# anonymousauthors001/SGS-GNN

Measured on AMD Instinct MI355X. Metric: sampled edges/sec + training steps/sec, Reddit hybrid 20% sparsity, higher is better.
Workload: dtype f32

## Files before the change

include/sgs_hip.h:

```cpp
#ifndef SGS_HIP_H_
#define SGS_HIP_H_

#include <stddef.h>
#include <stdint.h>

#ifdef __cplusplus
extern "C" {
#endif

#define SGS_ABI_VERSION 1

#define SGS_OK 0
#define SGS_EINVAL (-1)
#define SGS_EWORKSPACE (-2)
#define SGS_EHIP (-3)

typedef void* sgs_stream_t;

int sgs_abi_version(void);
const char* sgs_last_error(void);

int sgs_rng_set_epoch_buffer(const uint64_t* epoch_dev);
int sgs_exp_noise(uint64_t seed, uint64_t stream_id, int64_t E, float* noise, sgs_stream_t stream);
int sgs_dropout_keep(uint64_t seed, uint32_t site, int64_t rows, int64_t cols, float p, uint8_t* keep,
// ... 66 lines not shown

int sgs_gcn_norm_fwd(const float* w, int64_t n_edges, int64_t N, const int32_t* in_ptr, const int32_t* in_src,
                     const int32_t* in_eid, const int32_t* out_ptr, const int32_t* out_dst, const int32_t* out_eid,
                     const int32_t* loop_eid, float* dis, float* loopw, float* what_in, float* what_out,
                     float* what_loop, sgs_stream_t stream);

int sgs_gcn_degree_partial(const float* w, int64_t n_edges, int64_t N, const int32_t* in_ptr, const int32_t* in_src,
                           const int32_t* in_eid, float* degpart, sgs_stream_t stream);
int sgs_gcn_norm_from_degree(const float* w, const float* degsum, int64_t n_edges, int64_t N, const int32_t* in_ptr,
                             const int32_t* in_src, const int32_t* in_eid, const int32_t* out_ptr,
                             const int32_t* out_dst, const int32_t* out_eid, float* dis, float* loopw, float* what_in,
                             float* what_out, float* what_loop, sgs_stream_t stream);
int sgs_bias_act(const float* X, const float* bias, int64_t N, int64_t D, int act, float p_drop, uint64_t seed,
                 uint32_t site, float* Y, sgs_stream_t stream);
int sgs_bias_act_rows(const float* X, const float* bias, int64_t n_rows, int64_t D, int64_t row_offset, int act, float p_drop,
                      uint64_t seed, uint32_t site, float* Y, sgs_stream_t stream);

int sgs_mean_weights(int64_t n_edges, int64_t N, const int32_t* in_ptr, const int32_t* out_ptr, const int32_t* out_dst,
                     float* what_in, float* what_out, sgs_stream_t stream);
int sgs_degree_prior_logits(const int64_t* edge_index, int64_t E, int64_t N, const int32_t* in_ptr,
                            const int32_t* out_ptr, float* logits, sgs_stream_t stream);

size_t sgs_gcn_norm_bwd_workspace_bytes(int64_t N);
int sgs_gcn_norm_bwd(const float* w, const float* gw_hat, const float* gloop, int64_t n_edges, int64_t N,
                     const float* dis, const float* loopw, const int32_t* in_ptr, const int32_t* in_src,
                     const int32_t* in_eid, const int32_t* out_ptr, const int32_t* out_dst, const int32_t* out_eid,
                     const int32_t* loop_eid, const int64_t* edge_index, float* dw, void* ws, size_t ws_bytes,
                     sgs_stream_t stream);
int sgs_gcn_norm_bwd_sum(const float* w, const float* gw_hat, const float* gloop, const float* gw_hat2, const float* gloop2, const float* dw_add,
                         int64_t n_edges, int64_t N, const float* dis, const float* loopw, const int32_t* in_ptr, const int32_t* in_src,
                         const int32_t* in_eid, const int32_t* out_ptr, const int32_t* out_dst, const int32_t* out_eid,
                         const int32_t* loop_eid, const int64_t* edge_index, float* dw, void* ws, size_t ws_bytes, sgs_stream_t stream);

int sgs_gcn_norm_bwd_node(const float* w, const float* gw_hat, const float* gloop, int64_t n_edges, int64_t N,
                          const float* dis, const float* loopw, const int32_t* in_ptr, const int32_t* in_src,
                          const int32_t* in_eid, const int32_t* out_ptr, const int32_t* out_dst, const int32_t* out_eid,
                          float* Hn, sgs_stream_t stream);
int sgs_gcn_norm_bwd_edge(const float* gw_hat, const float* gloop, int64_t n_edges, int64_t N, const float* dis,
                          const int32_t* loop_eid, const int64_t* edge_index, const float* Hn, float* dw,
                          sgs_stream_t stream);

#define SGS_ACT_NONE 0
#define SGS_ACT_RELU 1
#define SGS_ACT_RELU_DROPOUT 2
int sgs_spmm_csr(const float* X, int64_t N, int64_t D, int64_t nnz, const int32_t* ptr, const int32_t* col, const float* val,
                 const float* diag, const float* bias, int act, float p_drop, uint64_t seed, uint32_t site, float* Y,
                 sgs_stream_t stream);

int sgs_sddmm_csr(const float* A, const float* B, int64_t N, int64_t D, int64_t nnz, const int32_t* ptr, const int32_t* col,
                  const int32_t* eid, float* g, float* gdiag, sgs_stream_t stream);

int sgs_spmm_csr_variant(int64_t N, int64_t D, int64_t nnz, int aligned16);
int sgs_sddmm_csr_variant(int64_t N, int64_t D, int64_t nnz, int aligned16);

int sgs_spmm_long_rows_set(int on);
int sgs_spmm_long_rows_threshold(void);
int sgs_spmm_long_rows_active(int64_t N, int64_t D);

int sgs_act_bwd(const float* dY, const float* Y, int64_t n, int act, float p_drop, float* dZ, sgs_stream_t stream);
size_t sgs_colsum_workspace_bytes(int64_t N, int64_t D);
int sgs_colsum(const float* A, int64_t N, int64_t D, float* out, void* ws, size_t ws_bytes, sgs_stream_t stream);
int sgs_act_bwd_colsum(const float* dY, const float* Y, int64_t N, int64_t D, int act, float p_drop, float* dZ, float* colsum, void* ws,
                       size_t ws_bytes, sgs_stream_t stream);

int sgs_colsum_variant(int64_t N, int64_t D, int fused_act);

int sgs_gcn_pair_ok(int64_t N, int64_t nnz, int64_t D);
int sgs_spmm_csr_next(const float* X, int64_t N, int64_t D, int64_t nnz, const int32_t* ptr, const int32_t* col, const float* val,
                      const float* diag, const float* bias, int act, float p_drop, uint64_t seed, uint32_t site, const float* Wn, int64_t Dn,
                      float* Y, float* Z, sgs_stream_t stream);
int sgs_spmm_csr_bwd_prev(const float* dZ, int64_t N, int64_t D, int64_t nnz, const int32_t* ptr, const int32_t* col, const float* val,
                          const float* diag, const float* W, int64_t Dp, const float* Yp, int act, float p_drop, float* dX, float* dZp,
                          float* colsum, sgs_stream_t stream);

int sgs_gcn_dual_ok(int64_t N, int64_t nnz_a, int64_t nnz_b, int64_t D, int64_t Dn);
int sgs_spmm_csr_next_dual(const float* X, int64_t N, int64_t D, const float* bias, int act, float p_drop, uint32_t site, const float* Wn,
                           int64_t Dn, int64_t nnz_a, const int32_t* ptr_a, const int32_t* col_a, const float* val_a, const float* diag_a,
                           uint64_t seed_a, float* Y_a, float* Z_a, int64_t nnz_b, const int32_t* ptr_b, const int32_t* col_b,
                           const float* val_b, const float* diag_b, uint64_t seed_b, float* Y_b, float* Z_b, sgs_stream_t stream);
int sgs_spmm_csr_dual(const float* X_a, const float* X_b, int64_t N, int64_t D, const float* bias, int act, float p_drop, uint32_t site,
                      int64_t nnz_a, const int32_t* ptr_a, const int32_t* col_a, const float* val_a, const float* diag_a, uint64_t seed_a,
                      float* Y_a, int64_t nnz_b, const int32_t* ptr_b, const int32_t* col_b, const float* val_b, const float* diag_b,
                      uint64_t seed_b, float* Y_b, sgs_stream_t stream);

size_t sgs_edge_score_workspace_bytes(int64_t N, int64_t H, int64_t E);
int sgs_edge_score_hidden_supported(int64_t H);
int sgs_edge_score_get_variant(void);
int sgs_edge_score_get_bwd_variant(void);
void sgs_edge_score_set_bwd_variant(int variant);
int sgs_edge_score_bwd_tile(void);
void sgs_edge_score_set_variant(int variant);
int sgs_edge_score_fwd(const float* codes, const float* U, int64_t N, int64_t H, const int64_t* edge_index, int64_t E,
                       int64_t edge_id_offset, const float* W1, const float* b1, const float* w2, const float* b2,
                       float p_drop, uint64_t seed, uint32_t site, float* p_out, void* ws, size_t ws_bytes,
                       sgs_stream_t stream);
size_t sgs_edge_mates_workspace_bytes(int64_t n_edges);
int sgs_edge_mates(const int64_t* edge_index, int64_t n_edges, int64_t N, const int32_t* out_ptr, const int32_t* out_dst,
                   const int32_t* out_eid, int32_t* mate, void* ws, size_t ws_bytes, sgs_stream_t stream);
int sgs_edge_score_paired_supported(int64_t H);
int sgs_edge_score_fwd_paired(const float* codes, const float* U, int64_t N, int64_t H, const int64_t* edge_index, int64_t E,
                              int64_t edge_id_offset, const int32_t* canon, int64_t M, const int32_t* mate, const float* W1, const float* b1,
                              const float* w2, const float* b2, float p_drop, uint64_t seed, uint32_t site, float* p_out, void* ws,
                              size_t ws_bytes, sgs_stream_t stream);
int sgs_edge_score_bwd_core(const float* codes, const float* U, int64_t N, int64_t H, const int64_t* edge_index,
                            int64_t E, int64_t edge_id_offset, const int64_t* active_eid, int64_t n_active, const float* grad_p,
                            const float* W1, const float* b1, const float* w2, const float* b2, float p_drop,
// ... 356 lines not shown
```

sgs-gnn_amd/csrc/gcn.hip:

```cpp
#include "sgs_common.h"

namespace sgs {
size_t graph_sort_workspace_bytes(int64_t n, int64_t N);
size_t graph_src_sorted_workspace_bytes(int64_t n, int64_t N);
int graph_build_src_sorted(const int64_t* ei, int64_t n, int64_t N, int32_t* in_ptr, int32_t* in_src, int32_t* in_eid, int32_t* out_ptr,
                           int32_t* out_dst, int32_t* out_eid, int32_t* loop_eid, int32_t* unsorted_flag, void* ws, size_t ws_bytes,
                           hipStream_t stream);
int graph_build_by_sort(const int64_t* ei, int64_t n, int64_t N, int32_t* in_ptr, int32_t* in_src, int32_t* in_eid, int32_t* out_ptr,
                        int32_t* out_dst, int32_t* out_eid, int32_t* loop_eid, void* ws, size_t ws_bytes, hipStream_t stream);
}

namespace sgs {
namespace {

constexpr int kT = 256;
constexpr int kMaxLdsRow = 8192;

__global__ void __launch_bounds__(kT) count_degrees(const int64_t* __restrict__ ei, int64_t n_edges, int* __restrict__ cnt_in,
                                                   int* __restrict__ cnt_out, int* __restrict__ loop_eid) {
    const int64_t e = static_cast<int64_t>(blockIdx.x) * kT + threadIdx.x;
    if (e >= n_edges) return;
    const int s = static_cast<int>(ei[e]), d = static_cast<int>(ei[n_edges + e]);
    atomicAdd(&cnt_in[d], 1);
    atomicAdd(&cnt_out[s], 1);
// ... 801 lines not shown
        float a[VEC];
#pragma unroll
        for (int v = 0; v < VEC; ++v) a[v] = 0.f;
        if (in) *reinterpret_cast<V*>(a) = *reinterpret_cast<const V*>(Ai + c0);
        const int64_t cl = in ? c0 : 0;
        for (int k = b + wave; k < e; k += 4 * NW) {
            int jc[4], ev[4];
#pragma unroll
            for (int u = 0; u < 4; ++u) {
                const int kk = k + NW * u;
                const int kc = kk < e ? kk : e - 1;
                jc[u] = col[kc];
                ev[u] = eid[kc];
            }
            float x[4][VEC];
#pragma unroll
            for (int u = 0; u < 4; ++u) *reinterpret_cast<V*>(x[u]) = *reinterpret_cast<const V*>(B + static_cast<int64_t>(jc[u]) * D + cl);
            float d[4];
#pragma unroll
            for (int u = 0; u < 4; ++u) {
                float acc = 0.f;
#pragma unroll
                for (int v = 0; v < VEC; ++v) acc = fmaf(a[v], in ? x[u][v] : 0.f, acc);
                d[u] = acc;
            }
#pragma unroll
            for (int u = 0; u < 4; ++u) d[u] = wave_sum_hi_dpp(d[u]);
            if (lane == 63) {
#pragma unroll
                for (int u = 0; u < 4; ++u)
                    if (k + NW * u < e) g[ev[u]] = d[u];
            }
        }
        if (wave == 0 && gdiag) {
            const float d0 = wave_sum_all(dot(i));
            if (lane == 0) gdiag[i] = d0;
        }
        return;
    }
    int k = b + wave;
    for (; k + NW < e; k += 2 * NW) {
        float d0 = dot(col[k]), d1 = dot(col[k + NW]);
#pragma unroll
        for (int o = 32; o > 0; o >>= 1) { d0 += __shfl_xor(d0, o, 64); d1 += __shfl_xor(d1, o, 64); }
        if (lane == 0) { g[eid[k]] = d0; g[eid[k + NW]] = d1; }
    }
    for (; k < e; k += NW) {
        const float d0 = wave_sum_all(dot(col[k]));
        if (lane == 0) g[eid[k]] = d0;
    }
    if (wave == 0 && gdiag) {
        const float d0 = wave_sum_all(dot(i));
        if (lane == 0) gdiag[i] = d0;
    }
}

__global__ void __launch_bounds__(kT) act_bwd(const float* __restrict__ dY, const float* __restrict__ Y, int64_t n, int act,
                                             float drop_scale, float* __restrict__ dZ) {
    const int64_t i = static_cast<int64_t>(blockIdx.x) * kT + threadIdx.x;
    if (i >= n) return;
    float g = dY[i];
    if (act != SGS_ACT_NONE) g = (Y[i] > 0.f) ? (act == SGS_ACT_RELU_DROPOUT ? g * drop_scale : g) : 0.f;
    dZ[i] = g;
}

constexpr int kColRows = 256;
inline int colsum_rows(int64_t N) { return N >= 16384 ? kColRows : (N >= 4096 ? 128 : 32); }
__global__ void __launch_bounds__(kT) colsum_partial(const float* __restrict__ A, int64_t N, int64_t D, int rows, float* __restrict__ part) {
    __shared__ float red[4][64];
    const int c = blockIdx.x * 64 + (threadIdx.x & 63);
    const int rgrp = threadIdx.x >> 6;
    const int64_t r0 = static_cast<int64_t>(blockIdx.y) * rows;
    const int64_t r1 = (r0 + rows < N) ? r0 + rows : N;
    float acc = 0.f;
    if (c < D)
        for (int64_t r = r0 + rgrp; r < r1; r += 4) acc += A[r * D + c];
    red[rgrp][threadIdx.x & 63] = acc;
    __syncthreads();
    if (rgrp == 0 && c < D)
        part[static_cast<int64_t>(blockIdx.y) * D + c] = (red[0][threadIdx.x] + red[1][threadIdx.x]) + (red[2][threadIdx.x] + red[3][threadIdx.x]);
}
template <int RG>
__global__ void __launch_bounds__(RG * 64) colsum_final(const float* __restrict__ part, int64_t nchunk, int64_t D, float* __restrict__ out) {
    __shared__ float red[RG][64];
    const int c = blockIdx.x * 64 + (threadIdx.x & 63);
    const int rgrp = threadIdx.x >> 6;
    float acc = 0.f;
    if (c < D)
        for (int64_t r = rgrp; r < nchunk; r += RG) acc += part[r * D + c];
    red[rgrp][threadIdx.x & 63] = acc;
    __syncthreads();
    if (rgrp == 0 && c < D) {
        float s = 0.f;
#pragma unroll
        for (int g = 0; g < RG; g += 4) s += (red[g][threadIdx.x] + red[g + 1][threadIdx.x]) + (red[g + 2][threadIdx.x] + red[g + 3][threadIdx.x]);
        out[c] = s;
    }
}

constexpr int kColSmallRows = 2048;
template <bool ACT>
__device__ __forceinline__ void colsum_small_body(const float* __restrict__ A, const float* __restrict__ Y, int64_t N, int64_t D, int act,
                                                  float drop_scale, float* __restrict__ dZ, float* __restrict__ out, int64_t blk) {
    __shared__ float red[64][17];
    const int cl = threadIdx.x & 15, rl = threadIdx.x >> 4;
    const int64_t c = blk * 16 + cl;
// ... 713 lines not shown
    const float scale = 1.0f / (1.0f - p_drop);
    const uint32_t th = dropout_thresh(p_drop);
    if (act == SGS_ACT_RELU_DROPOUT && p_drop == 0.f) act = SGS_ACT_RELU;
    const dim3 g_(static_cast<unsigned>(N));
    const bool lr = spmm_long_rows_on(N, D);
    switch (var) {
        case 1416:
            LAUNCH_LR(spmm_csr_rowblock, 4, 16, g_, dim3(1024), 0, stream, X, N, D, ptr, col, val, diag, bias, act, scale, th, seed,
                               site, epoch_ptr(), Y);
            break;
        case 1404:
            LAUNCH_LR(spmm_csr_rowblock, 4, 4, g_, dim3(kT), 0, stream, X, N, D, ptr, col, val, diag, bias, act, scale, th, seed,
                               site, epoch_ptr(), Y);
            break;
        case 1116:
            LAUNCH_LR(spmm_csr_rowblock, 1, 16, g_, dim3(1024), 0, stream, X, N, D, ptr, col, val, diag, bias, act, scale, th, seed,
                               site, epoch_ptr(), Y);
            break;
        case 1104:
            LAUNCH_LR(spmm_csr_rowblock, 1, 4, g_, dim3(kT), 0, stream, X, N, D, ptr, col, val, diag, bias, act, scale, th, seed,
                               site, epoch_ptr(), Y);
            break;
        default: {
            const int vec = var / 100, lpr = var % 100;
            DISPATCH_VEC_LPR(spmm_csr, vec, lpr, N, X, N, D, ptr, col, val, diag, bias, act, scale, th, seed, site, epoch_ptr(), Y);
        }
    }
    SGS_LAUNCH_OK();
    return SGS_OK;
}

int sgs_sddmm_csr(const float* A, const float* B, int64_t N, int64_t D, int64_t nnz, const int32_t* ptr, const int32_t* col,
                  const int32_t* eid, float* g, float* gdiag, sgs_stream_t stream_) {
    hipStream_t stream = static_cast<hipStream_t>(stream_);
    SGS_REQUIRE(N >= 0 && D >= 0, SGS_EINVAL, "sgs_sddmm_csr: bad sizes");
    if (N == 0) return SGS_OK;
    SGS_REQUIRE(A && B && ptr, SGS_EINVAL, "sgs_sddmm_csr: null pointer");
    const int var = sgs_sddmm_csr_variant(N, D, nnz, aligned16(A) && aligned16(B));
    const dim3 g_(static_cast<unsigned>(N));
    switch (var) {
        case 1416: hipLaunchKernelGGL((sddmm_csr_rowblock<4, 16>), g_, dim3(1024), 0, stream, A, B, N, D, ptr, col, eid, g, gdiag); break;
        case 1404: hipLaunchKernelGGL((sddmm_csr_rowblock<4, 4>), g_, dim3(kT), 0, stream, A, B, N, D, ptr, col, eid, g, gdiag); break;
        case 1116: hipLaunchKernelGGL((sddmm_csr_rowblock<1, 16>), g_, dim3(1024), 0, stream, A, B, N, D, ptr, col, eid, g, gdiag); break;
        case 1104: hipLaunchKernelGGL((sddmm_csr_rowblock<1, 4>), g_, dim3(kT), 0, stream, A, B, N, D, ptr, col, eid, g, gdiag); break;
        default: {
            const int vec = var / 100, lpr = var % 100;
            DISPATCH_VEC_LPR(sddmm_csr, vec, lpr, N, A, B, N, D, ptr, col, eid, g, gdiag);
        }
    }
    SGS_LAUNCH_OK();
    return SGS_OK;
}

int sgs_act_bwd(const float* dY, const float* Y, int64_t n, int act, float p_drop, float* dZ, sgs_stream_t stream_) {
    hipStream_t stream = static_cast<hipStream_t>(stream_);
    SGS_REQUIRE(n >= 0 && p_drop >= 0.f && p_drop < 1.f, SGS_EINVAL, "sgs_act_bwd: bad arguments");
    if (n == 0) return SGS_OK;
    SGS_REQUIRE(dY && dZ && (act == SGS_ACT_NONE || Y), SGS_EINVAL, "sgs_act_bwd: null pointer");
    if (act == SGS_ACT_RELU_DROPOUT && p_drop == 0.f) act = SGS_ACT_RELU;
    hipLaunchKernelGGL(act_bwd, dim3(cdiv(n, kT)), dim3(kT), 0, stream, dY, Y, n, act, 1.0f / (1.0f - p_drop), dZ);
    SGS_LAUNCH_OK();
    return SGS_OK;
}

size_t sgs_colsum_workspace_bytes(int64_t N, int64_t D) {
    if (N < 0) N = 0;
    if (D < 0) D = 0;
    return carve_bytes(static_cast<size_t>(cdiv(N, colsum_rows(N)) + 1) * D, 4) + 256;
}

int sgs_colsum_variant(int64_t N, int64_t D, int fused_act) {
    const int f = fused_act ? 100000 : 0;
    if (N > 0 && N <= kColSmallRows) return (D % 4 == 0 ? 2000000 : 1000000) + f;
    if (D == 1 && N > 0 && N <= kVecSumMax) return 3000000 + f;
    const int rows = colsum_rows(N);
    return 4000000 + f + rows * 100 + (cdiv(N, rows) > 64 ? 16 : 4);
}

int sgs_colsum(const float* A, int64_t N, int64_t D, float* out, void* ws, size_t ws_bytes, sgs_stream_t stream_) {
    hipStream_t stream = static_cast<hipStream_t>(stream_);
    SGS_REQUIRE(N >= 0 && D >= 0, SGS_EINVAL, "sgs_colsum: bad sizes");
    if (D == 0) return SGS_OK;
    SGS_REQUIRE(out && (N == 0 || A), SGS_EINVAL, "sgs_colsum: null pointer");
    SGS_REQUIRE(ws && ws_bytes >= sgs_colsum_workspace_bytes(N, D), SGS_EWORKSPACE, "sgs_colsum: workspace too small");
    const int var = sgs_colsum_variant(N, D, 0);
    switch (var / 1000000) {
        case 1:
            hipLaunchKernelGGL(colsum_small<false>, dim3(cdiv(D, 16)), dim3(1024), 0, stream, A, static_cast<const float*>(nullptr), N, D, SGS_ACT_NONE, 1.f,
                               static_cast<float*>(nullptr), out);
            break;
        case 2:
            hipLaunchKernelGGL(colsum_small_v4<false>, dim3(cdiv(D, 16)), dim3(1024), 0, stream, A, static_cast<const float*>(nullptr), N, D, SGS_ACT_NONE,
                               1.f, static_cast<float*>(nullptr), out);
            break;
        case 3:
            hipLaunchKernelGGL(vecsum_small, dim3(1), dim3(1024), 0, stream, A, N, out);
            break;
        default: {
            Carver cv(ws);
            const int rows = var / 100 % 1000;
            const int64_t nchunk = cdiv(N, rows);
            float* part = cv.take<float>(static_cast<size_t>(nchunk + 1) * D);
            if (nchunk > 0)
                hipLaunchKernelGGL(colsum_partial, dim3(cdiv(D, 64), nchunk), dim3(kT), 0, stream, A, N, D, rows, part);
            if (var % 100 == 16) hipLaunchKernelGGL(colsum_final<16>, dim3(cdiv(D, 64)), dim3(1024), 0, stream, part, nchunk, D, out);
            else                 hipLaunchKernelGGL(colsum_final<4>, dim3(cdiv(D, 64)), dim3(kT), 0, stream, part, nchunk, D, out);
// ... 277 lines not shown
```

sgs-gnn_amd/csrc/optim.hip:

```cpp
#include "sgs_common.h"

namespace sgs {
namespace {

constexpr int kAT = 256;
constexpr int kAChunk = 2048;
constexpr int kAMax = 24;

struct AdamDesc {
    float* p;
    const float* g;
    float* m;
    float* v;
    int64_t n;
    float* step;
    const float* gate;
};
struct AdamArgs {
    AdamDesc d[kAMax];
    int chunk_end[kAMax];
    int n_tensors;
    float lr, beta1, beta2, eps, weight_decay;
    int maximize;
    unsigned int* ticket;
};

__global__ void __launch_bounds__(kAT) adam_group(AdamArgs a) {
    __shared__ unsigned int s_last;
    int ti = 0;
    while (static_cast<int>(blockIdx.x) >= a.chunk_end[ti]) ++ti;
    const int chunk = static_cast<int>(blockIdx.x) - (ti ? a.chunk_end[ti - 1] : 0);
    const AdamDesc d = a.d[ti];
    const bool open = d.gate == nullptr || d.gate[0] != 0.f;
    const float t = d.step[0] + 1.0f;
    const double bc1 = 1.0 - exp(static_cast<double>(t) * log(static_cast<double>(a.beta1)));
    const double bc2 = 1.0 - exp(static_cast<double>(t) * log(static_cast<double>(a.beta2)));
    const float step_size = static_cast<float>(static_cast<double>(a.lr) / bc1);
    const float inv_sqrt_bc2 = static_cast<float>(1.0 / sqrt(bc2));
    const float beta1 = a.beta1, beta2 = a.beta2, eps = a.eps, wd = a.weight_decay;
    const int64_t base = static_cast<int64_t>(chunk) * kAChunk;
#pragma unroll
    for (int it = 0; it < kAChunk / kAT; ++it) {
        const int64_t i = base + static_cast<int64_t>(it) * kAT + threadIdx.x;
        if (open && i < d.n) {
            float g = d.g[i];
            if (a.maximize) g = -g;
            const float p = d.p[i];
            if (wd != 0.f) g = fmaf(wd, p, g);
            float m = d.m[i], v = d.v[i];
            m = m + (g - m) * (1.0f - beta1);
            v = beta2 * v + (1.0f - beta2) * g * g;
            const float denom = sqrtf(v) * inv_sqrt_bc2 + eps;
            d.m[i] = m;
            d.v[i] = v;
            d.p[i] = p - step_size * (m / denom);
        }
    }
    __syncthreads();
    if (threadIdx.x == 0) s_last = (atomicAdd(a.ticket, 1u) == gridDim.x - 1) ? 1u : 0u;
    __syncthreads();
    if (s_last) {
        if (static_cast<int>(threadIdx.x) < a.n_tensors) {
            const AdamDesc& dd = a.d[threadIdx.x];
            if (dd.gate == nullptr || dd.gate[0] != 0.f) dd.step[0] += 1.0f;
        }
        if (threadIdx.x == 0) __hip_atomic_store(a.ticket, 0u, __ATOMIC_RELAXED, __HIP_MEMORY_SCOPE_AGENT);
    }
}

constexpr int kAMax2 = 16;
struct AdamState {
    float* m;
    float* v;
    float* step;
    const float* gate;
    float lr, beta1, beta2, eps, wd;
    int maximize;
};
struct AdamDesc2 {
    float* p;
    const float* g;
    int64_t n;
    AdamState s[2];
    int n_states;
};
struct AdamArgs2 {
    AdamDesc2 d[kAMax2];
    int chunk_end[kAMax2];
    int n_tensors;
    unsigned int* ticket;
    float* loss_sum;
    const float* loss;
    unsigned long long* epoch;
};

__global__ void __launch_bounds__(kAT) adam_multi(AdamArgs2 a) {
    __shared__ unsigned int s_last;
    int ti = 0;
    while (static_cast<int>(blockIdx.x) >= a.chunk_end[ti]) ++ti;
    const int chunk = static_cast<int>(blockIdx.x) - (ti ? a.chunk_end[ti - 1] : 0);
    const AdamDesc2& d = a.d[ti];
    bool open[2];
    float step_size[2], inv_sqrt_bc2[2];
#pragma unroll
    for (int q = 0; q < 2; ++q) {
        open[q] = q < d.n_states && (d.s[q].gate == nullptr || d.s[q].gate[0] != 0.f);
        step_size[q] = 0.f;
        inv_sqrt_bc2[q] = 0.f;
        if (q < d.n_states) {
            const float t = d.s[q].step[0] + 1.0f;
            const double bc1 = 1.0 - exp(static_cast<double>(t) * log(static_cast<double>(d.s[q].beta1)));
            const double bc2 = 1.0 - exp(static_cast<double>(t) * log(static_cast<double>(d.s[q].beta2)));
            step_size[q] = static_cast<float>(static_cast<double>(d.s[q].lr) / bc1);
            inv_sqrt_bc2[q] = static_cast<float>(1.0 / sqrt(bc2));
        }
    }
    const int64_t base = static_cast<int64_t>(chunk) * kAChunk;
#pragma unroll
    for (int it = 0; it < kAChunk / kAT; ++it) {
        const int64_t i = base + static_cast<int64_t>(it) * kAT + threadIdx.x;
        if (i < d.n && (open[0] || open[1])) {
            const float g0 = d.g[i];
            float p = d.p[i];
#pragma unroll
            for (int q = 0; q < 2; ++q) {
                if (open[q]) {
                    const AdamState& st = d.s[q];
                    float g = st.maximize ? -g0 : g0;
                    if (st.wd != 0.f) g = fmaf(st.wd, p, g);
                    float m = st.m[i], v = st.v[i];
                    m = m + (g - m) * (1.0f - st.beta1);
                    v = st.beta2 * v + (1.0f - st.beta2) * g * g;
                    const float denom = sqrtf(v) * inv_sqrt_bc2[q] + st.eps;
                    st.m[i] = m;
                    st.v[i] = v;
                    p = p - step_size[q] * (m / denom);
                }
            }
            d.p[i] = p;
        }
    }
    __syncthreads();
    if (threadIdx.x == 0) s_last = (atomicAdd(a.ticket, 1u) == gridDim.x - 1) ? 1u : 0u;
    __syncthreads();
    if (s_last) {
        if (static_cast<int>(threadIdx.x) < 2 * a.n_tensors) {
            const AdamDesc2& dd = a.d[threadIdx.x >> 1];
            const int q = threadIdx.x & 1;
            if (q < dd.n_states && (dd.s[q].gate == nullptr || dd.s[q].gate[0] != 0.f)) {
                dd.s[q].step[0] += 1.0f;
            }
        }
        if (threadIdx.x == 64) {
            if (a.loss_sum && a.loss) a.loss_sum[0] += a.loss[0];
            if (a.epoch) a.epoch[0] += 1ull;
        }
        if (threadIdx.x == 0) __hip_atomic_store(a.ticket, 0u, __ATOMIC_RELAXED, __HIP_MEMORY_SCOPE_AGENT);
    }
}

}
}

using namespace sgs;

extern "C" {

int sgs_adam_max_tensors(void) { return kAMax; }

int sgs_adam_step(const int64_t* desc_host, int64_t n_tensors, float lr, float beta1, float beta2, float eps, float weight_decay,
                  int maximize, uint32_t* ticket, sgs_stream_t stream_) {
    hipStream_t stream = static_cast<hipStream_t>(stream_);
    SGS_REQUIRE(n_tensors >= 0 && n_tensors <= kAMax, SGS_EINVAL, "sgs_adam_step: at most %d tensors per call", kAMax);
    if (n_tensors == 0) return SGS_OK;
    SGS_REQUIRE(desc_host && ticket, SGS_EINVAL, "sgs_adam_step: null pointer");
    SGS_REQUIRE(beta1 >= 0.f && beta1 < 1.f && beta2 >= 0.f && beta2 < 1.f && eps >= 0.f, SGS_EINVAL, "sgs_adam_step: bad hyper-parameters");
    AdamArgs a{};
    int64_t total = 0;
    for (int i = 0; i < kAMax; ++i) {
        if (i < n_tensors) {
            const int64_t* w = desc_host + 7 * i;
            a.d[i].p = reinterpret_cast<float*>(w[0]);
            a.d[i].g = reinterpret_cast<const float*>(w[1]);
            a.d[i].m = reinterpret_cast<float*>(w[2]);
            a.d[i].v = reinterpret_cast<float*>(w[3]);
            a.d[i].n = w[4];
            a.d[i].step = reinterpret_cast<float*>(w[5]);
            a.d[i].gate = reinterpret_cast<const float*>(w[6]);
            SGS_REQUIRE(a.d[i].p && a.d[i].g && a.d[i].m && a.d[i].v && a.d[i].step && a.d[i].n >= 0, SGS_EINVAL,
                        "sgs_adam_step: bad descriptor %d", i);
            total += cdiv(a.d[i].n, kAChunk);
        }
        a.chunk_end[i] = static_cast<int>(total);
    }
// ... 59 lines not shown
```

sgs-gnn_amd/ops.py:

```python
from __future__ import annotations

import ctypes
import os
from typing import NamedTuple, Optional

import numpy as np
import torch

from . import _lib

SAMPLE_LEARNED, SAMPLE_PRIOR = 0, 1
ACT_NONE, ACT_RELU, ACT_RELU_DROPOUT = 0, 1, 2

_workspaces = {}
_retired_workspaces = []
_pin_workspaces = False


def _need_gpu(*tensors):
    for t in tensors:
        if t is not None and not t.is_cuda:
            raise RuntimeError("sgs_gnn_amd: the SGS hot path runs only on a HIP device (got a CPU tensor); "
                               "there is no CPU fallback")

# ... 1936 lines not shown
    return _leaf_dw(dY, x.contiguous(), x.shape[0], M, Nn, leaf=leaf)


class _GCNLayer(torch.autograd.Function):

    @staticmethod
    def forward(ctx, x, W, handle, bias, nm, act, p, seed, site, xl):
        gr = nm.graph
        if xl is None:
            xl = _x_wt(x, W)
        N, D = xl.shape
        Y = _spmm(xl, gr.in_ptr, gr.in_src, nm.what_in, nm.what_loop, bias, act, p, seed, site, N, D, gr.n_edges)
        ctx.nm, ctx.act, ctx.p = nm, act, p
        ctx.has_bias, ctx.has_handle = bias is not None, handle is not None
        ctx.save_for_backward(x, W, xl, Y if act != ACT_NONE else None)
        ctx.mark_non_differentiable(xl)
        ctx.set_materialize_grads(False)
        return Y, xl

    @staticmethod
    def backward(ctx, dY, _dxl_unused):
        L = _lib.lib()
        nm, gr = ctx.nm, ctx.nm.graph
        x, W, xl, Y = ctx.saved_tensors
        N, D = xl.shape
        dY = dY.contiguous()
        dx = dW = g = None
        want_db = ctx.has_bias and ctx.needs_input_grad[3]
        dZ, dbias = _grad_through_act(dY, Y, ctx.act, ctx.p, want_db, colsum_now=False)
        need_x, need_W = ctx.needs_input_grad[0], ctx.needs_input_grad[1]
        if need_x or need_W:
            dxl = _spmm(dZ, gr.out_ptr, gr.out_dst, nm.what_out, nm.what_loop, None, ACT_NONE, 0.0, 0, 0, N, D, gr.n_edges)
            if need_W:
                dW = _dyt_x(dxl, x, W.shape, leaf=(ctx, 1))
            if need_x:
                dx = dxl @ W
        if ctx.has_handle and ctx.needs_input_grad[2]:
            g = torch.empty(gr.n_edges + gr.N, dtype=torch.float32, device=dY.device)
            gw, gl = g[:gr.n_edges], g[gr.n_edges:]
            _lib.check(L.sgs_sddmm_csr(_ptr(dZ), _ptr(xl), N, D, gr.n_edges, _ptr(gr.in_ptr), _ptr(gr.in_src), _ptr(gr.in_eid),
                                       gw.data_ptr(), gl.data_ptr(), _stream()), "sgs_sddmm_csr")
        if want_db and dbias is None:
            dbias = _colsum(dZ)
        return dx, dW, (_handle_grad(nm, g) if g is not None else None), dbias, None, None, None, None, None, None


def gcn_layer(x, W, bias, nm: Norm, act=ACT_NONE, p=0.0, seed=0, site=0, xl=None):
    _need_gpu(x, W, bias)
    if x.dtype != torch.float32 or x.dim() != 2 or x.shape[0] != nm.graph.N:
        raise RuntimeError("gcn_layer: x must be float32 [N, F]")
    return _GCNLayer.apply(x, W, nm.handle, bias, nm, act, float(p), int(seed), int(site), xl)


def _pair_ok(gr, *widths):
    L = _lib.lib()
    return all(L.sgs_gcn_pair_ok(gr.N, gr.n_edges, int(w)) for w in widths)


class _GCN2(torch.autograd.Function):

    @staticmethod
    def forward(ctx, x, W1, b1, W2, b2, handle, nm, act, p, seed, site, xl1, pre=None):
        L = _lib.lib()
        gr = nm.graph
        if xl1 is None:
            xl1 = _x_wt(x, W1)
        N, H = xl1.shape
        C = W2.shape[0]
        fused = _pair_ok(gr, H, C) and xl1.is_contiguous() and W2.is_contiguous() and W2.shape[1] == H
        if pre is not None:
            h, xl2, out = pre
        elif fused:
            h = torch.empty(N, H, dtype=torch.float32, device=xl1.device)
            xl2 = torch.empty(N, C, dtype=torch.float32, device=xl1.device)
            _lib.check(L.sgs_spmm_csr_next(_ptr(xl1, torch.float32), N, H, gr.n_edges, _ptr(gr.in_ptr), _ptr(gr.in_src), _ptr(nm.what_in),
                                           _ptr(nm.what_loop), _ptr(b1), act, float(p), seed, site, _ptr(W2, torch.float32), C, _ptr(h),
                                           _ptr(xl2), _stream()), "sgs_spmm_csr_next")
        else:
            h = _spmm(xl1, gr.in_ptr, gr.in_src, nm.what_in, nm.what_loop, b1, act, p, seed, site, N, H, gr.n_edges)
            xl2 = h @ W2.t()
        if pre is None:
            out = _spmm(xl2, gr.in_ptr, gr.in_src, nm.what_in, nm.what_loop, b2, ACT_NONE, 0.0, 0, 0, N, C, gr.n_edges)
        ctx.nm, ctx.act, ctx.p, ctx.fused = nm, act, p, fused
        ctx.has_b1, ctx.has_b2, ctx.has_handle = b1 is not None, b2 is not None, handle is not None
        ctx.save_for_backward(x, W1, xl1, h, W2, xl2)
        ctx.mark_non_differentiable(xl1)
        ctx.set_materialize_grads(False)
        return out, xl1

    @staticmethod
    def backward(ctx, dout, _dxl_unused):
        L = _lib.lib()
        nm, gr = ctx.nm, ctx.nm.graph
        x, W1, xl1, h, W2, xl2 = ctx.saved_tensors
        N, H = h.shape
        C = W2.shape[0]
        need_x, need_W1, need_b1, need_W2, need_b2, need_g = (ctx.needs_input_grad[i] for i in range(6))
        need_b1, need_b2, need_g = need_b1 and ctx.has_b1, need_b2 and ctx.has_b2, need_g and ctx.has_handle
        dx = dW1 = db1 = dW2 = db2 = g = None
        dZ2 = dout.contiguous()
        f32 = dict(dtype=torch.float32, device=dZ2.device)

        def sddmm(dZ, xl, D):
            gg = torch.empty(gr.n_edges + gr.N, **f32)
            _lib.check(L.sgs_sddmm_csr(_ptr(dZ), _ptr(xl), N, D, gr.n_edges, _ptr(gr.in_ptr), _ptr(gr.in_src), _ptr(gr.in_eid),
                                       gg[:gr.n_edges].data_ptr(), gg[gr.n_edges:].data_ptr(), _stream()), "sgs_sddmm_csr")
            return gg

        want_1 = need_x or need_W1 or need_b1 or need_g
        dxl2 = dZ1 = None
        if want_1 or need_W2:
            dxl2 = torch.empty(N, C, **f32)
            if ctx.fused:
                dZ1 = torch.empty(N, H, **f32) if want_1 else None
                db2 = torch.empty(C, **f32) if need_b2 else None
                _lib.check(L.sgs_spmm_csr_bwd_prev(_ptr(dZ2), N, C, gr.n_edges, _ptr(gr.out_ptr), _ptr(gr.out_dst), _ptr(nm.what_out),
                                                   _ptr(nm.what_loop), _ptr(W2 if want_1 else None, torch.float32), H, _ptr(h), ctx.act,
                                                   float(ctx.p), _ptr(dxl2), _ptr(dZ1), _ptr(db2), _stream()), "sgs_spmm_csr_bwd_prev")
            else:
                dxl2 = _spmm(dZ2, gr.out_ptr, gr.out_dst, nm.what_out, nm.what_loop, None, ACT_NONE, 0.0, 0, 0, N, C, gr.n_edges)
        if need_W2:
            dW2 = _dyt_x(dxl2, h, W2.shape, leaf=(ctx, 3))
        if want_1 and not ctx.fused:
            dZ1h = dxl2 @ W2
            dZ1, db1 = _act_bwd_colsum(dZ1h, h, ctx.act, ctx.p) if need_b1 else (_act_bwd(dZ1h, h, ctx.act, ctx.p), None)
        g2 = sddmm(dZ2, xl2, C) if need_g else None
        if need_b2 and db2 is None:
            db2 = _colsum(dZ2)
        if need_x or need_W1 or (need_b1 and db1 is None and ctx.fused):
            if ctx.fused:
                dxl1 = torch.empty(N, H, **f32)
                db1 = torch.empty(H, **f32) if need_b1 else None
                _lib.check(L.sgs_spmm_csr_bwd_prev(_ptr(dZ1), N, H, gr.n_edges, _ptr(gr.out_ptr), _ptr(gr.out_dst), _ptr(nm.what_out),
                                                   _ptr(nm.what_loop), None, 0, None, ACT_NONE, 0.0, _ptr(dxl1), None, _ptr(db1), _stream()),
                           "sgs_spmm_csr_bwd_prev")
            else:
                dxl1 = _spmm(dZ1, gr.out_ptr, gr.out_dst, nm.what_out, nm.what_loop, None, ACT_NONE, 0.0, 0, 0, N, H, gr.n_edges)
            if need_W1:
                dW1 = _dyt_x(dxl1, x, W1.shape, leaf=(ctx, 1))
            if need_x:
                dx = dxl1 @ W1
        g1 = sddmm(dZ1, xl1, H) if need_g else None
        if need_b1 and db1 is None:
            db1 = _colsum(dZ1)
        if need_g:
            r2, r1 = _handle_grad(nm, g2), _handle_grad(nm, g1)
            g = r2 if r1 is None else (r1 if r2 is None else r2 + r1)
        return dx, dW1, db1, dW2, db2, g, None, None, None, None, None, None, None


def gcn2(x, W1, b1, W2, b2, nm: Norm, act=ACT_RELU, p=0.0, seed=0, site=0, xl1=None):
    _need_gpu(x, W1, b1, W2, b2)
    if x.dtype != torch.float32 or x.dim() != 2 or x.shape[0] != nm.graph.N:
        raise RuntimeError("gcn2: x must be float32 [N, F]")
    return _GCN2.apply(x, W1, b1, W2, b2, nm.handle, nm, act, float(p), int(seed), int(site), xl1)


_gcn_dual_enabled = True
GCN_DUAL_FORWARDS = {"shared": 0}


def set_gcn_dual(on: bool) -> None:
    global _gcn_dual_enabled
    _gcn_dual_enabled = bool(on)


def gcn_dual_enabled() -> bool:
    return _gcn_dual_enabled


def gcn_dual_ok(gr_a, gr_b, H: int, C: int) -> bool:
    return (gr_a.N == gr_b.N and bool(_lib.lib().sgs_gcn_dual_ok(gr_a.N, gr_a.n_edges, gr_b.n_edges, int(H), int(C)))
            and _pair_ok(gr_a, H, C) and _pair_ok(gr_b, H, C))


def _gcn2_dual_forward(xl1, b1, W2, b2, nm_a, nm_b, act, p, seed_a, seed_b, site):
    L = _lib.lib()
    GCN_DUAL_FORWARDS["shared"] += 1
    ga, gb = nm_a.graph, nm_b.graph
    N, H = xl1.shape
    C = W2.shape[0]
    f32 = dict(dtype=torch.float32, device=xl1.device)
    h_a, xl2_a, out_a = torch.empty(N, H, **f32), torch.empty(N, C, **f32), torch.empty(N, C, **f32)
    h_b, xl2_b, out_b = torch.empty(N, H, **f32), torch.empty(N, C, **f32), torch.empty(N, C, **f32)
    _lib.check(L.sgs_spmm_csr_next_dual(_ptr(xl1, torch.float32), N, H, _ptr(b1), act, float(p), site, _ptr(W2, torch.float32), C,
                                        ga.n_edges, _ptr(ga.in_ptr), _ptr(ga.in_src), _ptr(nm_a.what_in), _ptr(nm_a.what_loop), seed_a,
                                        _ptr(h_a), _ptr(xl2_a),
                                        gb.n_edges, _ptr(gb.in_ptr), _ptr(gb.in_src), _ptr(nm_b.what_in), _ptr(nm_b.what_loop), seed_b,
                                        _ptr(h_b), _ptr(xl2_b), _stream()), "sgs_spmm_csr_next_dual")
    _lib.check(L.sgs_spmm_csr_dual(_ptr(xl2_a), _ptr(xl2_b), N, C, _ptr(b2), ACT_NONE, 0.0, 0,
                                   ga.n_edges, _ptr(ga.in_ptr), _ptr(ga.in_src), _ptr(nm_a.what_in), _ptr(nm_a.what_loop), 0, _ptr(out_a),
                                   gb.n_edges, _ptr(gb.in_ptr), _ptr(gb.in_src), _ptr(nm_b.what_in), _ptr(nm_b.what_loop), 0, _ptr(out_b),
                                   _stream()), "sgs_spmm_csr_dual")
    return (h_a, xl2_a, out_a), (h_b, xl2_b, out_b)


def gcn2_dual(x, W1, b1, W2, b2, nm_a: Norm, nm_b: Norm, act=ACT_RELU, p=0.0, seed_a=0, seed_b=0, site=0, xl1=None):
    _need_gpu(x, W1, b1, W2, b2)
# ... 382 lines not shown
```

Measured before the change: 111.1 million.

## Fuse two-layer SDDMM edge gradients into one kernel and vectorize Adam updates

Adds a paired SDDMM kernel that computes both layers' edge-weight gradients in one pass over the CSR structure. It gathers the neighbor rows for both layers per edge and writes the summed dot products, replacing two launches, two index traversals and a later elementwise add. Separately, the Adam kernels are restructured around a shared chunk routine that uses float4 loads and stores when pointers are aligned and the chunk is full. The fused path only applies under size and alignment conditions and raises register pressure per thread.

```diff
diff --git a/include/sgs_hip.h b/include/sgs_hip.h
--- a/include/sgs_hip.h
+++ b/include/sgs_hip.h
@@ -142,6 +142,10 @@
 
 int sgs_spmm_csr_variant(int64_t N, int64_t D, int64_t nnz, int aligned16);
 int sgs_sddmm_csr_variant(int64_t N, int64_t D, int64_t nnz, int aligned16);
+
+int sgs_sddmm_csr_pair_ok(int64_t N, int64_t nnz, int64_t D1, int64_t D2, int aligned16);
+int sgs_sddmm_csr_pair(const float* A1, const float* B1, int64_t D1, const float* A2, const float* B2, int64_t D2, int64_t N, int64_t nnz,
+                       const int32_t* ptr, const int32_t* col, const int32_t* eid, float* g, float* gdiag, sgs_stream_t stream);
 
 int sgs_spmm_long_rows_set(int on);
 int sgs_spmm_long_rows_threshold(void);
diff --git a/sgs-gnn_amd/csrc/gcn.hip b/sgs-gnn_amd/csrc/gcn.hip
--- a/sgs-gnn_amd/csrc/gcn.hip
+++ b/sgs-gnn_amd/csrc/gcn.hip
@@ -877,6 +877,74 @@
     if (wave == 0 && gdiag) {
         const float d0 = wave_sum_all(dot(i));
         if (lane == 0) gdiag[i] = d0;
+    }
+}
+
+template <int NW, int V2>
+__global__ void __launch_bounds__(64 * NW) sddmm_csr_rowblock_pair(const float* __restrict__ A1, const float* __restrict__ B1, int64_t D1,
+                                                             const float* __restrict__ A2, const float* __restrict__ B2, int64_t D2,
+                                                             const int* __restrict__ ptr, const int* __restrict__ col,
+                                                             const int* __restrict__ eid, float* __restrict__ g, float* __restrict__ gdiag) {
+    using W2 = typename VecT<V2>::type;
+    const int lane = threadIdx.x & 63, wave = threadIdx.x >> 6;
+    const int64_t i = blockIdx.x;
+    const int b = ptr[i], e = ptr[i + 1];
+    const int64_t c1 = static_cast<int64_t>(lane) * 4, c2 = static_cast<int64_t>(lane) * V2;
+    const bool in1 = c1 < D1, in2 = c2 < D2;
+    const int64_t cl1 = in1 ? c1 : 0, cl2 = in2 ? c2 : 0;
+    float a1[4], a2[V2];
+#pragma unroll
+    for (int v = 0; v < 4; ++v) a1[v] = 0.f;
+#pragma unroll
+    for (int v = 0; v < V2; ++v) a2[v] = 0.f;
+    if (in1) *reinterpret_cast<float4*>(a1) = *reinterpret_cast<const float4*>(A1 + i * D1 + c1);
+    if (in2) *reinterpret_cast<W2*>(a2) = *reinterpret_cast<const W2*>(A2 + i * D2 + c2);
+    for (int k = b + wave; k < e; k += 4 * NW) {
+        int jc[4], ev[4];
+#pragma unroll
+        for (int u = 0; u < 4; ++u) {
+            const int kk = k + NW * u;
+            const int kc = kk < e ? kk : e - 1;
+            jc[u] = col[kc];
+            ev[u] = eid[kc];
+        }
+        float x1[4][4], x2[4][V2];
+#pragma unroll
+        for (int u = 0; u < 4; ++u) *reinterpret_cast<float4*>(x1[u]) = *reinterpret_cast<const float4*>(B1 + static_cast<int64_t>(jc[u]) * D1 + cl1);
+#pragma unroll
+        for (int u = 0; u < 4; ++u) *reinterpret_cast<W2*>(x2[u]) = *reinterpret_cast<const W2*>(B2 + static_cast<int64_t>(jc[u]) * D2 + cl2);
+        float d1[4], d2[4];
+#pragma unroll
+        for (int u = 0; u < 4; ++u) {
+            float acc = 0.f;
+#pragma unroll
+            for (int v = 0; v < 4; ++v) acc = fmaf(a1[v], in1 ? x1[u][v] : 0.f, acc);
+            d1[u] = acc;
+            acc = 0.f;
+#pragma unroll
+            for (int v = 0; v < V2; ++v) acc = fmaf(a2[v], in2 ? x2[u][v] : 0.f, acc);
+            d2[u] = acc;
+        }
+#pragma unroll
+        for (int u = 0; u < 4; ++u) { d1[u] = wave_sum_hi_dpp(d1[u]); d2[u] = wave_sum_hi_dpp(d2[u]); }
+        if (lane == 63) {
+#pragma unroll
+            for (int u = 0; u < 4; ++u)
+                if (k + NW * u < e) g[ev[u]] = d1[u] + d2[u];
+        }
+    }
+    if (wave == 0 && gdiag) {
+        float x1[4], x2[V2];
+        *reinterpret_cast<float4*>(x1) = *reinterpret_cast<const float4*>(B1 + i * D1 + cl1);
+        *reinterpret_cast<W2*>(x2) = *reinterpret_cast<const W2*>(B2 + i * D2 + cl2);
+        float s1 = 0.f, s2 = 0.f;
+#pragma unroll
+        for (int v = 0; v < 4; ++v) s1 = fmaf(a1[v], in1 ? x1[v] : 0.f, s1);
+#pragma unroll
+        for (int v = 0; v < V2; ++v) s2 = fmaf(a2[v], in2 ? x2[v] : 0.f, s2);
+        s1 = wave_sum_all(s1);
+        s2 = wave_sum_all(s2);
+        if (lane == 0) gdiag[i] = s1 + s2;
     }
 }
 
@@ -1696,6 +1764,33 @@
     return SGS_OK;
 }
 
+int sgs_sddmm_csr_pair_ok(int64_t N, int64_t nnz, int64_t D1, int64_t D2, int aligned16_) {
+    return N > 0 && N < (int64_t(1) << 31) && nnz >= 16 * N
+           && D1 > 0 && D1 <= 256 && D1 % 4 == 0 && aligned16_
+           && D2 > 0 && D2 <= 64;
+}
+
+int sgs_sddmm_csr_pair(const float* A1, const float* B1, int64_t D1, const float* A2, const float* B2, int64_t D2, int64_t N, int64_t nnz,
+                       const int32_t* ptr, const int32_t* col, const int32_t* eid, float* g, float* gdiag, sgs_stream_t stream_) {
+    hipStream_t stream = static_cast<hipStream_t>(stream_);
+    SGS_REQUIRE(N >= 0 && D1 >= 0 && D2 >= 0, SGS_EINVAL, "sgs_sddmm_csr_pair: bad sizes");
+    if (N == 0) return SGS_OK;
+    SGS_REQUIRE(A1 && B1 && A2 && B2 && ptr && col && eid && g, SGS_EINVAL, "sgs_sddmm_csr_pair: null pointer");
+    SGS_REQUIRE(sgs_sddmm_csr_pair_ok(N, nnz, D1, D2, aligned16(A1) && aligned16(B1)), SGS_EINVAL,
+                "sgs_sddmm_csr_pair: needs nnz >= 16 N, D1 %% 4 == 0, D1 <= 256, 16-byte aligned A1 / B1 and 0 < D2 <= 64 "
+                "(N %lld, nnz %lld, D1 %lld, D2 %lld): make the two sgs_sddmm_csr calls",
+                static_cast<long long>(N), static_cast<long long>(nnz), static_cast<long long>(D1), static_cast<long long>(D2));
+    const int v1 = sgs_sddmm_csr_variant(N, D1, nnz, 1), v2 = sgs_sddmm_csr_variant(N, D2, nnz, aligned16(A2) && aligned16(B2));
+    const bool w16 = v1 % 100 == 16, vec2 = v2 / 100 % 10 == 4;
+    const dim3 g_(static_cast<unsigned>(N));
+    if (w16 && vec2) hipLaunchKernelGGL((sddmm_csr_rowblock_pair<16, 4>), g_, dim3(1024), 0, stream, A1, B1, D1, A2, B2, D2, ptr, col, eid, g, gdiag);
+    else if (w16) hipLaunchKernelGGL((sddmm_csr_rowblock_pair<16, 1>), g_, dim3(1024), 0, stream, A1, B1, D1, A2, B2, D2, ptr, col, eid, g, gdiag);
+    else if (vec2) hipLaunchKernelGGL((sddmm_csr_rowblock_pair<4, 4>), g_, dim3(kT), 0, stream, A1, B1, D1, A2, B2, D2, ptr, col, eid, g, gdiag);
+    else hipLaunchKernelGGL((sddmm_csr_rowblock_pair<4, 1>), g_, dim3(kT), 0, stream, A1, B1, D1, A2, B2, D2, ptr, col, eid, g, gdiag);
+    SGS_LAUNCH_OK();
+    return SGS_OK;
+}
+
 int sgs_act_bwd(const float* dY, const float* Y, int64_t n, int act, float p_drop, float* dZ, sgs_stream_t stream_) {
     hipStream_t stream = static_cast<hipStream_t>(stream_);
     SGS_REQUIRE(n >= 0 && p_drop >= 0.f && p_drop < 1.f, SGS_EINVAL, "sgs_act_bwd: bad arguments");
diff --git a/sgs-gnn_amd/csrc/optim.hip b/sgs-gnn_amd/csrc/optim.hip
--- a/sgs-gnn_amd/csrc/optim.hip
+++ b/sgs-gnn_amd/csrc/optim.hip
@@ -24,6 +24,88 @@
     int maximize;
     unsigned int* ticket;
 };
+
+struct AdamCoef {
+    float* m;
+    float* v;
+    float beta1, beta2, eps, wd, step_size, inv_sqrt_bc2;
+    bool maximize, open;
+};
+template <int VEC> struct AdamVec;
+template <> struct AdamVec<1> { using type = float; };
+template <> struct AdamVec<4> { using type = float4; };
+
+template <int VEC>
+__device__ __forceinline__ void adam_chunk(float* p_, const float* g_, int64_t n, int64_t base, const AdamCoef (&c)[2]) {
+    using V = typename AdamVec<VEC>::type;
+    constexpr int K = kAChunk / (kAT * VEC);
+    int64_t at[K];
+    bool live[K];
+    float g0[K][VEC], p[K][VEC], m[2][K][VEC], v[2][K][VEC];
+#pragma unroll
+    for (int k = 0; k < K; ++k) {
+        const int64_t i = base + (static_cast<int64_t>(k) * kAT + threadIdx.x) * VEC;
+        live[k] = VEC == 4 || i < n;
+        at[k] = live[k] ? i : n - 1;
+    }
+#pragma unroll
+    for (int k = 0; k < K; ++k) *reinterpret_cast<V*>(g0[k]) = *reinterpret_cast<const V*>(g_ + at[k]);
+#pragma unroll
+    for (int k = 0; k < K; ++k) *reinterpret_cast<V*>(p[k]) = *reinterpret_cast<const V*>(p_ + at[k]);
+#pragma unroll
+    for (int q = 0; q < 2; ++q) {
+        if (c[q].open) {
+#pragma unroll
+            for (int k = 0; k < K; ++k) *reinterpret_cast<V*>(m[q][k]) = *reinterpret_cast<const V*>(c[q].m + at[k]);
+#pragma unroll
+            for (int k = 0; k < K; ++k) *reinterpret_cast<V*>(v[q][k]) = *reinterpret_cast<const V*>(c[q].v + at[k]);
+        }
+    }
+#pragma unroll
+    for (int q = 0; q < 2; ++q) {
+        if (c[q].open) {
+#pragma unroll
+            for (int k = 0; k < K; ++k) {
+#pragma unroll
+                for (int e = 0; e < VEC; ++e) {
+                    float g = c[q].maximize ? -g0[k][e] : g0[k][e];
+                    if (c[q].wd != 0.f) g = fmaf(c[q].wd, p[k][e], g);
+                    float mm = m[q][k][e], vv = v[q][k][e];
+                    mm = mm + (g - mm) * (1.0f - c[q].beta1);
+                    vv = c[q].beta2 * vv + (1.0f - c[q].beta2) * g * g;
+                    const float denom = sqrtf(vv) * c[q].inv_sqrt_bc2 + c[q].eps;
+                    m[q][k][e] = mm;
+                    v[q][k][e] = vv;
+                    p[k][e] = p[k][e] - c[q].step_size * (mm / denom);
+                }
+            }
+        }
+    }
+#pragma unroll
+    for (int q = 0; q < 2; ++q) {
+        if (c[q].open) {
+#pragma unroll
+            for (int k = 0; k < K; ++k) {
+                if (live[k]) {
+                    *reinterpret_cast<V*>(c[q].m + at[k]) = *reinterpret_cast<const V*>(m[q][k]);
+                    *reinterpret_cast<V*>(c[q].v + at[k]) = *reinterpret_cast<const V*>(v[q][k]);
+                }
+            }
+        }
+    }
+#pragma unroll
+    for (int k = 0; k < K; ++k)
+        if (live[k]) *reinterpret_cast<V*>(p_ + at[k]) = *reinterpret_cast<const V*>(p[k]);
+}
+
+__device__ __forceinline__ void adam_chunk_any(float* p, const float* g, int64_t n, int64_t base, const AdamCoef (&c)[2]) {
+    uintptr_t bits = reinterpret_cast<uintptr_t>(p) | reinterpret_cast<uintptr_t>(g);
+#pragma unroll
+    for (int q = 0; q < 2; ++q)
+        if (c[q].open) bits |= reinterpret_cast<uintptr_t>(c[q].m) | reinterpret_cast<uintptr_t>(c[q].v);
+    if ((bits & 15) == 0 && base + kAChunk <= n) adam_chunk<4>(p, g, n, base, c);
+    else adam_chunk<1>(p, g, n, base, c);
+}
 
 __global__ void __launch_bounds__(kAT) adam_group(AdamArgs a) {
     __shared__ unsigned int s_last;
@@ -35,27 +117,13 @@
     const float t = d.step[0] + 1.0f;
     const double bc1 = 1.0 - exp(static_cast<double>(t) * log(static_cast<double>(a.beta1)));
     const double bc2 = 1.0 - exp(static_cast<double>(t) * log(static_cast<double>(a.beta2)));
-    const float step_size = static_cast<float>(static_cast<double>(a.lr) / bc1);
-    const float inv_sqrt_bc2 = static_cast<float>(1.0 / sqrt(bc2));
-    const float beta1 = a.beta1, beta2 = a.beta2, eps = a.eps, wd = a.weight_decay;
-    const int64_t base = static_cast<int64_t>(chunk) * kAChunk;
-#pragma unroll
-    for (int it = 0; it < kAChunk / kAT; ++it) {
-        const int64_t i = base + static_cast<int64_t>(it) * kAT + threadIdx.x;
-        if (open && i < d.n) {
-            float g = d.g[i];
-            if (a.maximize) g = -g;
-            const float p = d.p[i];
-            if (wd != 0.f) g = fmaf(wd, p, g);
-            float m = d.m[i], v = d.v[i];
-            m = m + (g - m) * (1.0f - beta1);
-            v = beta2 * v + (1.0f - beta2) * g * g;
-            const float denom = sqrtf(v) * inv_sqrt_bc2 + eps;
-            d.m[i] = m;
-            d.v[i] = v;
-            d.p[i] = p - step_size * (m / denom);
-        }
-    }
+    AdamCoef c[2] = {};
+    c[0].m = d.m; c[0].v = d.v;
+    c[0].beta1 = a.beta1; c[0].beta2 = a.beta2; c[0].eps = a.eps; c[0].wd = a.weight_decay;
+    c[0].step_size = static_cast<float>(static_cast<double>(a.lr) / bc1);
+    c[0].inv_sqrt_bc2 = static_cast<float>(1.0 / sqrt(bc2));
+    c[0].maximize = a.maximize != 0; c[0].open = open;
+    if (open) adam_chunk_any(d.p, d.g, d.n, static_cast<int64_t>(chunk) * kAChunk, c);
     __syncthreads();
     if (threadIdx.x == 0) s_last = (atomicAdd(a.ticket, 1u) == gridDim.x - 1) ? 1u : 0u;
     __syncthreads();
@@ -100,46 +168,23 @@
     while (static_cast<int>(blockIdx.x) >= a.chunk_end[ti]) ++ti;
     const int chunk = static_cast<int>(blockIdx.x) - (ti ? a.chunk_end[ti - 1] : 0);
     const AdamDesc2& d = a.d[ti];
-    bool open[2];
-    float step_size[2], inv_sqrt_bc2[2];
-#pragma unroll
-    for (int q = 0; q < 2; ++q) {
-        open[q] = q < d.n_states && (d.s[q].gate == nullptr || d.s[q].gate[0] != 0.f);
-        step_size[q] = 0.f;
-        inv_sqrt_bc2[q] = 0.f;
+    AdamCoef c[2] = {};
+#pragma unroll
+    for (int q = 0; q < 2; ++q) {
+        c[q].open = q < d.n_states && (d.s[q].gate == nullptr || d.s[q].gate[0] != 0.f);
         if (q < d.n_states) {
-            const float t = d.s[q].step[0] + 1.0f;
-            const double bc1 = 1.0 - exp(static_cast<double>(t) * log(static_cast<double>(d.s[q].beta1)));
-            const double bc2 = 1.0 - exp(static_cast<double>(t) * log(static_cast<double>(d.s[q].beta2)));
-            step_size[q] = static_cast<float>(static_cast<double>(d.s[q].lr) / bc1);
-            inv_sqrt_bc2[q] = static_cast<float>(1.0 / sqrt(bc2));
-        }
-    }
-    const int64_t base = static_cast<int64_t>(chunk) * kAChunk;
-#pragma unroll
-    for (int it = 0; it < kAChunk / kAT; ++it) {
-        const int64_t i = base + static_cast<int64_t>(it) * kAT + threadIdx.x;
-        if (i < d.n && (open[0] || open[1])) {
-            const float g0 = d.g[i];
-            float p = d.p[i];
-#pragma unroll
-            for (int q = 0; q < 2; ++q) {
-                if (open[q]) {
-                    const AdamState& st = d.s[q];
-                    float g = st.maximize ? -g0 : g0;
-                    if (st.wd != 0.f) g = fmaf(st.wd, p, g);
-                    float m = st.m[i], v = st.v[i];
-                    m = m + (g - m) * (1.0f - st.beta1);
-                    v = st.beta2 * v + (1.0f - st.beta2) * g * g;
-                    const float denom = sqrtf(v) * inv_sqrt_bc2[q] + st.eps;
-                    st.m[i] = m;
-                    st.v[i] = v;
-                    p = p - step_size[q] * (m / denom);
-                }
-            }
-            d.p[i] = p;
-        }
-    }
+            const AdamState& st = d.s[q];
+            const float t = st.step[0] + 1.0f;
+            const double bc1 = 1.0 - exp(static_cast<double>(t) * log(static_cast<double>(st.beta1)));
+            const double bc2 = 1.0 - exp(static_cast<double>(t) * log(static_cast<double>(st.beta2)));
+            c[q].step_size = static_cast<float>(static_cast<double>(st.lr) / bc1);
+            c[q].inv_sqrt_bc2 = static_cast<float>(1.0 / sqrt(bc2));
+            c[q].m = st.m; c[q].v = st.v;
+            c[q].beta1 = st.beta1; c[q].beta2 = st.beta2; c[q].eps = st.eps; c[q].wd = st.wd;
+            c[q].maximize = st.maximize != 0;
+        }
+    }
+    if (c[0].open || c[1].open) adam_chunk_any(d.p, d.g, d.n, static_cast<int64_t>(chunk) * kAChunk, c);
     __syncthreads();
     if (threadIdx.x == 0) s_last = (atomicAdd(a.ticket, 1u) == gridDim.x - 1) ? 1u : 0u;
     __syncthreads();
diff --git a/sgs-gnn_amd/ops.py b/sgs-gnn_amd/ops.py
--- a/sgs-gnn_amd/ops.py
+++ b/sgs-gnn_amd/ops.py
@@ -2012,6 +2012,19 @@
     return _GCNLayer.apply(x, W, nm.handle, bias, nm, act, float(p), int(seed), int(site), xl)
 
 
+_sddmm_pair_enabled = True
+SDDMM_PAIR_LAUNCHES = {"pair": 0}
+
+
+def set_sddmm_pair(on: bool) -> None:
+    global _sddmm_pair_enabled
+    _sddmm_pair_enabled = bool(on)
+
+
+def sddmm_pair_enabled() -> bool:
+    return _sddmm_pair_enabled
+
+
 def _pair_ok(gr, *widths):
     L = _lib.lib()
     return all(L.sgs_gcn_pair_ok(gr.N, gr.n_edges, int(w)) for w in widths)
@@ -2084,7 +2097,10 @@
         if want_1 and not ctx.fused:
             dZ1h = dxl2 @ W2
             dZ1, db1 = _act_bwd_colsum(dZ1h, h, ctx.act, ctx.p) if need_b1 else (_act_bwd(dZ1h, h, ctx.act, ctx.p), None)
-        g2 = sddmm(dZ2, xl2, C) if need_g else None
+        pair = (need_g and _sddmm_pair_enabled and dZ1 is not None and dZ1.is_contiguous() and xl1.is_contiguous() and xl2.is_contiguous()
+                and not (nm._park_ok and (nm._g_first is not None or nm._g_extra is not None))
+                and bool(L.sgs_sddmm_csr_pair_ok(N, gr.n_edges, H, C, int(dZ1.data_ptr() % 16 == 0 and xl1.data_ptr() % 16 == 0))))
+        g2 = sddmm(dZ2, xl2, C) if need_g and not pair else None
         if need_b2 and db2 is None:
             db2 = _colsum(dZ2)
         if need_x or need_W1 or (need_b1 and db1 is None and ctx.fused):
@@ -2100,10 +2116,18 @@
                 dW1 = _dyt_x(dxl1, x, W1.shape, leaf=(ctx, 1))
             if need_x:
                 dx = dxl1 @ W1
-        g1 = sddmm(dZ1, xl1, H) if need_g else None
+        g1 = sddmm(dZ1, xl1, H) if need_g and not pair else None
+        if pair:
+            gs = torch.empty(gr.n_edges + gr.N, **f32)
+            _lib.check(L.sgs_sddmm_csr_pair(_ptr(dZ1), _ptr(xl1), H, _ptr(dZ2), _ptr(xl2), C, N, gr.n_edges, _ptr(gr.in_ptr), _ptr(gr.in_src),
+                                            _ptr(gr.in_eid), gs[:gr.n_edges].data_ptr(), gs[gr.n_edges:].data_ptr(), _stream()),
+                       "sgs_sddmm_csr_pair")
+            SDDMM_PAIR_LAUNCHES["pair"] += 1
         if need_b1 and db1 is None:
             db1 = _colsum(dZ1)
-        if need_g:
+        if pair:
+            g = _handle_grad(nm, gs)
+        elif need_g:
             r2, r1 = _handle_grad(nm, g2), _handle_grad(nm, g1)
             g = r2 if r1 is None else (r1 if r2 is None else r2 + r1)
         return dx, dW1, db1, dW2, db2, g, None, None, None, None, None, None, None
```

After: 113.2 million, median of 3. Within noise of the previous version (+1.9%).
